# DIG-Beihang/RobustART

Measured on AMD Instinct MI355X. Metric: corrupted+attacked images/sec/node (ResNet-50, PGD-7 + IN-C x5), higher is better.
Workload: dtype bf16x3; 1 GPU; per step and GPU: gaussian_noise sev 1..5 on 256 u8 224x224 images -> normalise -> ResNet-50 eval (1280 img) + PGD-Linf-7 eps 2/255 ResNet-50 eval (256 img); global_batch=256, parallelism=dp1, streams=2

## Files before the change

### include/robustart_hip.h

```cpp
#ifndef ROBUSTART_HIP_H
#define ROBUSTART_HIP_H

#include <stddef.h>
#include <stdint.h>

#ifdef __cplusplus
extern "C" {
#endif

typedef void* rart_stream_t;

typedef enum rart_status {
  RART_OK = 0,
  RART_ERR_INVALID = 1,
  RART_ERR_UNSUPPORTED = 2,
  RART_ERR_WORKSPACE = 3,
  RART_ERR_HIP = 4
} rart_status;

enum {
  RART_GAUSSIAN_NOISE = 0, RART_SHOT_NOISE = 1, RART_IMPULSE_NOISE = 2, RART_DEFOCUS_BLUR = 3,
  RART_GLASS_BLUR = 4, RART_MOTION_BLUR = 5, RART_ZOOM_BLUR = 6, RART_SNOW = 7, RART_FROST = 8,
  RART_FOG = 9, RART_BRIGHTNESS = 10, RART_CONTRAST = 11, RART_ELASTIC_TRANSFORM = 12,
  RART_PIXELATE = 13, RART_JPEG_COMPRESSION = 14, RART_SPECKLE_NOISE = 15, RART_GAUSSIAN_BLUR = 16,
// ... 117 lines not shown
                      float* delta_u, int rows, size_t n, rart_stream_t stream);
int rart_row_count_diff(const float* a, const float* b, float* out, int rows, size_t n, rart_stream_t stream);

int rart_select_rows(float* dst, const float* src, const uint8_t* mask, int batch, size_t n_per_sample,
                     rart_stream_t stream);

int rart_logit_loss(const float* logits, const int64_t* y, const int64_t* y_target, int batch, int classes,
                    int kind, float scale, float* loss_out, float* dlogits_out, int32_t* pred_out,
                    rart_stream_t stream);

typedef struct rart_conv_desc {
  const void* src;
  const void* wgt;
  const float* bias;
  const void* res;
  const void* mask;
  void* dst;
  int32_t batch, grid_h, grid_w;
  int32_t src_h, src_w, src_pix_stride;
  int32_t k_per_tap, n_taps;
  int32_t sy, sx;
  int32_t tap_dy[32], tap_dx[32];
  int64_t tap_src_off[32];
  int32_t n_cols;
  int32_t dst_h, dst_w, dst_sy, dst_sx, dst_oy, dst_ox, dst_pix_stride;
  int32_t flags;
  int32_t n_batched, z_inner, wgt_row_stride, reserved_;
  int64_t src_z_outer, src_z_inner, wgt_z_outer, wgt_z_inner, dst_z_outer, dst_z_inner;
  void* sign_out;
  int64_t dst_pair_off, res_pair_off;
  float* bn_stats_out;
} rart_conv_desc;

int rart_conv_igemm_bf16(const rart_conv_desc* desc_host, rart_stream_t stream);
int rart_igemm_set_bk64_min_k(long long k);
int rart_gemm_small_m_bf16(const void* a, int lda, const void* w, int ldw, const float* bias, void* out, int ldo, int out_is_f32, int m,
                           int n, int k, rart_stream_t stream);
int rart_igemm_set_gemm256(int enable);
int rart_gemm256_supported(long long rows, int k, int n_cols, int src_ld, int dst_ld);

typedef struct rart_gemm_pair_desc {
  const void *a_hi, *a_lo, *w_hi, *w_lo;
  const float* bias;
  const void *res_hi, *res_lo;
  void *dst_hi, *dst_lo;
  void *aux_hi, *aux_lo;
  int M, N, K, lda, ldw, ldc, w_rows;
  int rows_per_image, src_rows_per_image, src_row_off, dst_rows_per_image, dst_row_off;
  int flags, n_batched, z_inner;
  int64_t a_z_outer, a_z_inner, w_z_outer, w_z_inner, c_z_outer, c_z_inner;
  int conv, batch, grid_h, grid_w, src_h, src_w, sy, sx, k_per_tap, n_taps;
  int tap_dy[16], tap_dx[16];
  int dst_h, dst_w, dst_sy, dst_sx, dst_oy, dst_ox;
  const void* mask_bits;
  void* sign_out;
  int tile_n;
  int tile_m;
} rart_gemm_pair_desc;
int rart_gemm_pair_bf16(const rart_gemm_pair_desc* desc_host, rart_stream_t stream);
int rart_gemm_pair_set_schedule(int mode);
int rart_gemm_pair_get_schedule(void);

typedef struct rart_conv_tail_desc {
  const void* a_hi;  const void* a_lo;
  const void* w_hi;  const void* w_lo;
  const void* t_hi;  const void* t_lo;
  const float* bias_mid;
  const float* bias_out;
  const void* mask_mid;  const void* mask_out;
  void* sign_mid;  void* sign_out;
  const void* res_hi;  const void* res_lo;
  void* dst_hi;  void* dst_lo;
  int batch, h, w, c_mid, ldw, relu_mid, relu_out;
  int tap_dy[9], tap_dx[9];
  const void* n_hi;  const void* n_lo;
  const float* bias_next;
  const void* mask_next;
  void* sign_next;
  void* dstn_hi;  void* dstn_lo;
  int relu_next;
} rart_conv_tail_desc;
int rart_conv3x3_tail_pair_supported(int c_mid);
int rart_conv3x3_tail_pair(const rart_conv_tail_desc* desc_host, rart_stream_t stream);

int rart_vit_add_pos_cls_pair(void* x_hi, void* x_lo, const float* cls_pos0, const float* pos, int n, int tokens, int dim,
                              rart_stream_t stream);
int rart_layernorm_pair(const void* x_hi, const void* x_lo, const float* gamma, const float* beta, void* out_hi, void* out_lo, int rows,
                        int dim, int64_t in_row_stride, int64_t out_row_stride, float eps, rart_stream_t stream);
int rart_layernorm_bwd_pair(const void* dy_hi, const void* dy_lo, const void* x_hi, const void* x_lo, const float* gamma,
                            const void* res_hi, const void* res_lo, void* dx_hi, void* dx_lo, int rows, int dim, int64_t dy_row_stride,
                            int64_t x_row_stride, int64_t res_row_stride, int64_t dx_row_stride, float eps, rart_stream_t stream);
int rart_softmax_rows_pair(const float* scores, void* probs_hi, void* probs_lo, int64_t rows, int n_valid, int ld_in, int ld_out,
                           float scale, rart_stream_t stream);
int rart_softmax_bwd_rows_pair(const void* probs_hi, const void* probs_lo, const float* dprobs, void* ds_hi, void* ds_lo, int64_t rows,
                               int n_valid, int ld_p, int ld_dp, int ld_out, float scale, rart_stream_t stream);
int rart_vit_unpatchify_from_f32(const float* dpatches, float* grad, int n, int h, int w, int patch, int64_t ld, const float* std_host,
                                 rart_stream_t stream);
int rart_vit_attention_pair(const void* qkv_hi, const void* qkv_lo, void* out_hi, void* out_lo, int n, int tokens, int heads, int head_dim,
                            rart_stream_t stream);
int rart_vit_attention_bwd_pair(const void* qkv_hi, const void* qkv_lo, const void* out_hi, const void* out_lo, const void* dout_hi,
                                const void* dout_lo, void* dqkv_hi, void* dqkv_lo, float* stats, int n, int tokens, int heads, int head_dim,
                                rart_stream_t stream);

int rart_conv3x3_halo_supported(int channels, int h, int w);
int rart_conv3x3_pack_frag_bf16(const void* w_rows, void* w_frag, int channels, rart_stream_t stream);
int rart_pack_frag_bf16(const void* w_rows, void* w_frag, int rows, int k, rart_stream_t stream);
int rart_conv3x3_halo_bf16(const void* src, const void* wgt, const float* bias, const void* mask_bits, void* sign_out,
                           void* dst, int n, int h, int w, int channels, const int* tap_dy, const int* tap_dx, int relu,
                           rart_stream_t stream);

int rart_bottleneck_fused_supported(int c_io, int c_mid, int h, int w);
int rart_bottleneck_fused_bf16(const void* x, const void* w1, const void* w2, const void* w3, const float* b1, const float* b2,
                               const float* b3, void* m1, void* m2, void* m3, void* out, int n, int h, int w, int c_io,
                               int c_mid, const int* tap_dy, const int* tap_dx, int backward, rart_stream_t stream);

int rart_bottleneck_first_supported(int c_in, int c_mid, int c_out, int h, int w);
int rart_bottleneck_first_bf16(const void* x, const void* w1, const void* w2, const void* w3, const void* w4, const float* b1,
                               const float* b2, const float* b3, void* m1, void* m2, void* m3, void* out, int n, int h, int w,
                               int c_in, int c_mid, int c_out, const int* tap_dy, const int* tap_dx, int backward,
                               rart_stream_t stream);

int rart_bottleneck_s2_fwd_supported(int c_in, int c_mid, int c_out, int h, int w);
int rart_bottleneck_s2_fwd_bf16(const void* x, const void* w1, const void* w2, const void* w3, const void* wd, const float* b1,
                                const float* b2, const float* b3, void* m1, void* m2, void* m3, void* out, int n, int h, int w,
                                int c_in, int c_mid, int c_out, rart_stream_t stream);

int rart_bottleneck_s2_bwd_bf16(const void* g, const void* w3t, const void* w2t, const void* w1t, const void* wdt, const void* m2,
                                const void* m1, const void* m0, void* dx, int n, int h, int w, int c_in, int c_mid, int c_out,
                                rart_stream_t stream);

int rart_bottleneck14_fused_supported(int c_io, int c_mid, int h, int w);
int rart_bottleneck14_fused_bf16(const void* x, const void* w1, const void* w2, const void* w3, const float* b1, const float* b2,
                                 const float* b3, void* m1, void* m2, void* m3, void* out, int n, int h, int w, int c_io,
                                 int c_mid, const int* tap_dy, const int* tap_dx, int backward, rart_stream_t stream);

int rart_bottleneck28_fused_supported(int c_io, int c_mid, int h, int w);
int rart_bottleneck28_fused_bf16(const void* x, const void* w1, const void* w2, const void* w3, const float* b1, const float* b2,
                                 const float* b3, void* m1, void* m2, void* m3, void* out, int n, int h, int w, int c_io,
                                 int c_mid, const int* tap_dy, const int* tap_dx, int backward, rart_stream_t stream);

int rart_bottleneck7_fused_supported(int c_io, int c_mid, int h, int w);
int rart_bottleneck7_fused_bf16(const void* x, const void* w1, const void* w2, const void* w3, const float* b1, const float* b2,
                                const float* b3, void* m1, void* m2, void* m3, void* out, int n, int h, int w, int c_io,
                                int c_mid, const int* tap_dy, const int* tap_dx, int backward, rart_stream_t stream);

int rart_engine_prep_input(const void* src, int src_is_u8, void* hi, void* lo, int n, int h, int w,
                           const float* mean_host, const float* std_host, rart_stream_t stream);
int rart_engine_maxpool(const void* in, void* out, void* argmax_out, int n, int h, int w, int c,
                        rart_stream_t stream);
int rart_engine_maxpool_keep(const void* in, void* out, void* argmax_out, void* sign_out, int n, int h, int w, int c,
                             rart_stream_t stream);
int rart_engine_maxpool_bwd(const void* y, const void* argmax, const void* dpool, void* dz, int n, int h, int w,
                            int c, rart_stream_t stream);
int rart_engine_avgpool(const void* in, void* out, int n, int hw, int c, rart_stream_t stream);
int rart_engine_avgpool_bwd(const void* y, const void* dpool, void* dz, int n, int hw, int c, rart_stream_t stream);
int rart_engine_stem_col2im(const void* patches, float* grad, int n, int h, int w, int patch_cols,
                            const float* std_host, rart_stream_t stream);
int rart_engine_maxpool_pair(const void* in_hi, long long in_lo_off, void* out_hi, long long out_lo_off, void* argmax_out,
                             void* sign_out, int n, int h, int w, int c, rart_stream_t stream);
int rart_engine_maxpool_bwd_pair(const void* argmax, const void* dpool_hi, long long dpool_lo_off, void* dz_hi,
                                 long long dz_lo_off, int n, int h, int w, int c, rart_stream_t stream);
int rart_engine_avgpool_pair(const void* in_hi, long long in_lo_off, void* out_hi, long long out_lo_off, int n, int hw, int c,
                             rart_stream_t stream);
int rart_engine_avgpool_bwd_pair(const void* y_sign_bits, const void* dpool_hi, long long dpool_lo_off, void* dz_hi,
                                 long long dz_lo_off, int n, int hw, int c, rart_stream_t stream);
int rart_f32_to_pair_rows(const float* src, void* dst_hi, long long dst_lo_off, int rows, int cols, int dst_cols,
// ... 132 lines not shown
```

### robustart_amd/_lib.py

```python
import ctypes
import os

_HERE = os.path.dirname(os.path.abspath(__file__))
LIB_PATH = os.path.join(_HERE, 'lib', 'librobustart_hip.so')

c_void_p, c_int, c_size_t, c_u64, c_float = (ctypes.c_void_p, ctypes.c_int, ctypes.c_size_t,
                                              ctypes.c_uint64, ctypes.c_float)
c_double = ctypes.c_double

ABI_VERSION = 110

SIGNATURES = {
    'rart_version': (c_int, []),
    'rart_last_error_string': (ctypes.c_char_p, []),
    'rart_corruption_name': (ctypes.c_char_p, [c_int]),
    'rart_corrupt_workspace_bytes': (c_size_t, [c_int, c_int, c_int, c_int, c_int]),
    'rart_corrupt_u8': (c_int, [c_void_p, c_void_p, c_int, c_int, c_int, c_int, c_int, c_u64, c_u64,
                                ctypes.POINTER(c_void_p), c_int, c_void_p, c_size_t, c_void_p]),
    'rart_stencil_fixed_point_info': (c_int, [c_int, c_int, c_void_p, c_void_p, c_size_t]),
    'rart_noise_multi_u8': (c_int, [c_void_p, ctypes.POINTER(c_void_p), c_int, c_int, c_int, c_int, c_int, ctypes.POINTER(c_int),
                                    ctypes.POINTER(c_u64), c_u64, c_void_p]),
    'rart_frost_textures_u8': (c_int, [c_void_p, c_void_p, c_int, c_int, c_int, c_int, c_void_p, c_int, c_int, c_int, ctypes.POINTER(c_int),
                                       c_u64, c_u64, c_void_p]),
    'rart_pil_resize_workspace_bytes': (c_size_t, [c_int] * 10),
# ... 23 lines not shown
                               c_void_p, c_void_p, c_size_t, c_void_p]),
    'rart_apgd_step': (c_int, [c_void_p, c_void_p, c_void_p, c_void_p, c_void_p, c_int, c_size_t, c_int,
                               c_float, c_float, c_void_p, c_size_t, c_void_p]),
    'rart_square_init_linf': (c_int, [c_void_p, c_void_p, c_int, c_int, c_int, c_int, c_float, c_u64, c_u64, c_void_p, c_void_p,
                                      c_void_p]),
    'rart_rng_signs_f32': (c_int, [c_void_p, c_int, c_int, c_u64, c_u64, c_void_p, c_int, ctypes.c_uint32, c_void_p]),
    'rart_rng_normal_rows_f32': (c_int, [c_void_p, c_int, c_size_t, c_u64, c_void_p, c_int, c_void_p]),
    'rart_square_propose_linf': (c_int, [c_void_p, c_void_p, c_void_p, c_int, c_int, c_int, c_int, c_float, c_int, c_int,
                                         c_int, c_void_p, c_void_p]),
    'rart_fab_project_linf': (c_int, [c_void_p, c_void_p, c_void_p, c_void_p, c_void_p, c_int, c_size_t, c_void_p]),
    'rart_row_dot': (c_int, [c_void_p, c_void_p, c_void_p, c_int, c_size_t, c_void_p]),
    'rart_row_absmax_diff': (c_int, [c_void_p, c_void_p, c_void_p, c_int, c_size_t, c_void_p]),
    'rart_eot_accumulate': (c_int, [c_void_p, c_void_p, c_size_t, c_int, c_float, c_void_p]),
    'rart_square_init_lp': (c_int, [c_void_p, c_void_p, c_int, c_int, c_int, c_int, c_float, c_int, c_int, c_int, c_int, c_int, c_void_p,
                                    c_void_p, c_void_p, c_void_p]),
    'rart_square_propose_lp': (c_int, [c_void_p, c_void_p, c_void_p, c_int, c_int, c_int, c_int, c_float, c_int, c_int, c_int, c_int, c_int,
                                       c_int, c_void_p, c_void_p, c_void_p]),
    'rart_fab_project': (c_int, [c_void_p, c_void_p, c_void_p, c_void_p, c_void_p, c_int, c_size_t, c_int, c_void_p]),
    'rart_row_norm_diff': (c_int, [c_void_p, c_void_p, c_void_p, c_int, c_size_t, c_int, c_void_p]),
    'rart_fab_update': (c_int, [c_void_p, c_void_p, c_void_p, c_void_p, c_void_p, c_int, c_size_t, c_float, c_void_p]),
    'rart_fab_backoff': (c_int, [c_void_p, c_void_p, c_void_p, c_int, c_size_t, c_float, c_void_p]),
    'rart_l1_project': (c_int, [c_void_p, c_void_p, c_void_p, c_int, c_size_t, c_float, c_int, c_int, c_void_p]),
    'rart_row_kth_abs': (c_int, [c_void_p, c_void_p, c_void_p, c_int, c_size_t, c_void_p]),
    'rart_apgd_l1_move': (c_int, [c_void_p, c_void_p, c_void_p, c_void_p, c_void_p, c_void_p, c_int, c_size_t, c_void_p]),
    'rart_row_count_diff': (c_int, [c_void_p, c_void_p, c_void_p, c_int, c_size_t, c_void_p]),
    'rart_select_rows': (c_int, [c_void_p, c_void_p, c_void_p, c_int, c_size_t, c_void_p]),
    'rart_logit_loss': (c_int, [c_void_p, c_void_p, c_void_p, c_int, c_int, c_int, c_float, c_void_p,
                                c_void_p, c_void_p, c_void_p]),
    'rart_conv_igemm_bf16': (c_int, [c_void_p, c_void_p]),
    'rart_conv3x3_halo_supported': (c_int, [c_int, c_int, c_int]),
    'rart_conv3x3_pack_frag_bf16': (c_int, [c_void_p, c_void_p, c_int, c_void_p]),
    'rart_pack_frag_bf16': (c_int, [c_void_p, c_void_p, c_int, c_int, c_void_p]),
    'rart_conv3x3_halo_bf16': (c_int, [c_void_p, c_void_p, c_void_p, c_void_p, c_void_p, c_void_p, c_int, c_int, c_int, c_int,
                                       ctypes.POINTER(c_int), ctypes.POINTER(c_int), c_int, c_void_p]),
    'rart_bottleneck28_fused_supported': (c_int, [c_int, c_int, c_int, c_int]),
    'rart_bottleneck28_fused_bf16': (c_int, [c_void_p] * 11 + [c_int] * 5 + [ctypes.POINTER(c_int), ctypes.POINTER(c_int), c_int,
                                             c_void_p]),
    'rart_bottleneck7_fused_supported': (c_int, [c_int, c_int, c_int, c_int]),
    'rart_bottleneck7_fused_bf16': (c_int, [c_void_p] * 11 + [c_int] * 5 + [ctypes.POINTER(c_int), ctypes.POINTER(c_int), c_int,
                                            c_void_p]),
    'rart_bottleneck_s2_fwd_supported': (c_int, [c_int] * 5),
    'rart_bottleneck_s2_fwd_bf16': (c_int, [c_void_p] * 12 + [c_int] * 6 + [c_void_p]),
    'rart_bottleneck_s2_bwd_bf16': (c_int, [c_void_p] * 9 + [c_int] * 6 + [c_void_p]),
    'rart_bottleneck14_fused_supported': (c_int, [c_int, c_int, c_int, c_int]),
    'rart_bottleneck14_fused_bf16': (c_int, [c_void_p] * 11 + [c_int] * 5 + [ctypes.POINTER(c_int), ctypes.POINTER(c_int), c_int,
                                             c_void_p]),
    'rart_bottleneck_fused_supported': (c_int, [c_int, c_int, c_int, c_int]),
    'rart_bottleneck_first_supported': (c_int, [c_int] * 5),
    'rart_bottleneck_first_bf16': (c_int, [c_void_p] * 12 + [c_int] * 6 + [ctypes.POINTER(c_int), ctypes.POINTER(c_int), c_int,
                                           c_void_p]),
    'rart_bottleneck_fused_bf16': (c_int, [c_void_p] * 11 + [c_int] * 5 + [ctypes.POINTER(c_int), ctypes.POINTER(c_int), c_int,
                                           c_void_p]),
    'rart_igemm_set_bk64_min_k': (c_int, [ctypes.c_longlong]),
    'rart_gemm_small_m_bf16': (c_int, [c_void_p, c_int, c_void_p, c_int, c_void_p, c_void_p, c_int, c_int, c_int, c_int, c_int, c_void_p]),
    'rart_igemm_set_gemm256': (c_int, [c_int]),
    'rart_gemm256_supported': (c_int, [ctypes.c_longlong, c_int, c_int, c_int, c_int]),
    'rart_gemm_pair_bf16': (c_int, [c_void_p, c_void_p]),
    'rart_copy_calibration': (c_int, [c_void_p, c_void_p, ctypes.c_size_t, c_int, c_void_p]),
    'rart_gemm_pair_set_schedule': (c_int, [c_int]),
    'rart_gemm_pair_get_schedule': (c_int, []),
    'rart_pack_jobs_bf16': (c_int, [c_void_p, c_int, c_int, c_void_p]),
    'rart_vit_add_pos_cls_pair': (c_int, [c_void_p, c_void_p, c_void_p, c_void_p, c_int, c_int, c_int, c_void_p]),
    'rart_layernorm_pair': (c_int, [c_void_p] * 6 + [c_int, c_int, ctypes.c_int64, ctypes.c_int64, c_float, c_void_p]),
    'rart_layernorm_bwd_pair': (c_int, [c_void_p] * 9 + [c_int, c_int] + [ctypes.c_int64] * 4 + [c_float, c_void_p]),
    'rart_softmax_rows_pair': (c_int, [c_void_p, c_void_p, c_void_p, ctypes.c_int64, c_int, c_int, c_int, c_float, c_void_p]),
    'rart_softmax_bwd_rows_pair': (c_int, [c_void_p] * 5 + [ctypes.c_int64, c_int, c_int, c_int, c_int, c_float, c_void_p]),
    'rart_vit_attention_pair': (c_int, [c_void_p, c_void_p, c_void_p, c_void_p, c_int, c_int, c_int, c_int, c_void_p]),
    'rart_vit_attention_bwd_pair': (c_int, [c_void_p] * 9 + [c_int, c_int, c_int, c_int, c_void_p]),
    'rart_vit_unpatchify_from_f32': (c_int, [c_void_p, c_void_p, c_int, c_int, c_int, c_int, ctypes.c_int64, ctypes.POINTER(c_float), c_void_p]),
    'rart_engine_prep_input': (c_int, [c_void_p, c_int, c_void_p, c_void_p, c_int, c_int, c_int, c_void_p, c_void_p,
                                       c_void_p]),
    'rart_engine_maxpool': (c_int, [c_void_p, c_void_p, c_void_p, c_int, c_int, c_int, c_int, c_void_p]),
    'rart_engine_maxpool_keep': (c_int, [c_void_p, c_void_p, c_void_p, c_void_p, c_int, c_int, c_int, c_int, c_void_p]),
    'rart_engine_maxpool_bwd': (c_int, [c_void_p, c_void_p, c_void_p, c_void_p, c_int, c_int, c_int, c_int, c_void_p]),
    'rart_engine_avgpool': (c_int, [c_void_p, c_void_p, c_int, c_int, c_int, c_void_p]),
    'rart_engine_avgpool_bwd': (c_int, [c_void_p, c_void_p, c_void_p, c_int, c_int, c_int, c_void_p]),
    'rart_engine_stem_col2im': (c_int, [c_void_p, c_void_p, c_int, c_int, c_int, c_int, c_void_p, c_void_p]),
    'rart_engine_stem_fwd_fused': (c_int, [c_void_p, c_int, c_void_p, c_int, c_void_p, c_void_p, c_void_p, c_void_p, c_int, c_int,
                                           c_int, c_void_p, c_void_p, c_void_p]),
    'rart_wgrad_direct_supported': (c_int, [c_int, c_int, c_int]),
    'rart_wgrad_direct_bf16': (c_int, [c_void_p, c_void_p, c_void_p] + [c_int] * 10 + [c_void_p, c_void_p, c_int, c_int, c_int, c_void_p]),
    'rart_conv3x3_tail_pair_supported': (c_int, [c_int]),
    'rart_conv3x3_tail_pair': (c_int, [c_void_p, c_void_p]),
    'rart_engine_stem_fwd_fused_pair': (c_int, [c_void_p, c_int] + [c_void_p] * 7 + [c_int, c_int, c_int, c_void_p, c_void_p, c_void_p]),
    'rart_engine_stem_bwd_fused_pair': (c_int, [c_void_p] * 6 + [c_int, c_int, c_int, c_void_p, c_void_p]),
    'rart_engine_stem_bwd_fused': (c_int, [c_void_p, c_void_p, c_void_p, c_void_p, c_int, c_int, c_int, c_void_p, c_void_p]),
    'rart_engine_maxpool_pair': (c_int, [c_void_p, ctypes.c_longlong, c_void_p, ctypes.c_longlong, c_void_p, c_void_p, c_int, c_int, c_int, c_int, c_void_p]),
    'rart_engine_maxpool_bwd_pair': (c_int, [c_void_p, c_void_p, ctypes.c_longlong, c_void_p, ctypes.c_longlong, c_int, c_int, c_int, c_int, c_void_p]),
    'rart_engine_avgpool_pair': (c_int, [c_void_p, ctypes.c_longlong, c_void_p, ctypes.c_longlong, c_int, c_int, c_int, c_void_p]),
    'rart_engine_avgpool_bwd_pair': (c_int, [c_void_p, c_void_p, ctypes.c_longlong, c_void_p, ctypes.c_longlong, c_int, c_int, c_int, c_void_p]),
    'rart_f32_to_pair_rows': (c_int, [c_void_p, c_void_p, ctypes.c_longlong, c_int, c_int, c_int, c_void_p]),
    'rart_engine_stem_col2im_f32': (c_int, [c_void_p, c_void_p, c_int, c_int, c_int, c_int, c_void_p, c_void_p]),
    'rart_f32_to_bf16_rows': (c_int, [c_void_p, c_void_p, c_int, c_int, c_int, c_void_p]),
    'rart_cnx_dwconv_ln_bf16': (c_int, [c_void_p] * 7 + [c_int] * 4 + [c_float, c_void_p]),
    'rart_cnx_dwconv_ln_pair': (c_int, [c_void_p] * 10 + [c_int] * 4 + [c_float, c_void_p]),
    'rart_cnx_dwconv_bwd_bf16': (c_int, [c_void_p] * 4 + [c_int] * 4 + [c_void_p]),
    'rart_cnx_dwconv_bwd_pair': (c_int, [c_void_p] * 7 + [c_int] * 4 + [c_void_p]),
    'rart_cnx_pool_bwd_bf16': (c_int, [c_void_p, c_void_p, c_int, c_int, c_int, c_void_p]),
    'rart_cnx_pool_bwd_pair': (c_int, [c_void_p] * 4 + [c_int, c_int, c_int, c_void_p]),
    'rart_cnx_patchify': (c_int, [c_void_p, c_int, c_void_p, c_void_p, c_int, c_int, c_int, c_int, c_int, c_void_p, c_void_p, c_void_p]),
    'rart_cnx_dwconv_wgrad_workspace_bytes': (c_size_t, [c_int] * 4),
    'rart_cnx_dwconv_wgrad_bf16': (c_int, [c_void_p] * 4 + [c_int] * 6 + [c_void_p, c_size_t, c_void_p]),
    'rart_cnx_layer_scale_fwd_bf16': (c_int, [c_void_p] * 4 + [ctypes.c_longlong, c_int, c_void_p]),
    'rart_cnx_layer_scale_bwd_workspace_bytes': (c_size_t, [ctypes.c_longlong, c_int]),
    'rart_cnx_layer_scale_bwd_bf16': (c_int, [c_void_p] * 6 + [ctypes.c_longlong, c_int, c_int, c_void_p, c_size_t, c_void_p]),
    'rart_cnx_grn_stats_bf16': (c_int, [c_void_p] * 2 + [c_int] * 3 + [c_void_p]),
    'rart_cnx_grn_stats_pair': (c_int, [c_void_p] * 3 + [c_int] * 3 + [c_void_p]),
    'rart_cnx_grn_apply_bf16': (c_int, [c_void_p] * 5 + [c_int] * 3 + [c_float, c_void_p]),
    'rart_cnx_grn_apply_pair': (c_int, [c_void_p] * 7 + [c_int] * 3 + [c_float, c_void_p]),
    'rart_cnx_grn_bwd_reduce_bf16': (c_int, [c_void_p] * 4 + [c_int] * 3 + [c_void_p]),
    'rart_cnx_grn_bwd_reduce_pair': (c_int, [c_void_p] * 6 + [c_int] * 3 + [c_void_p]),
    'rart_cnx_grn_bwd_apply_bf16': (c_int, [c_void_p] * 7 + [c_int] * 3 + [c_float, c_void_p]),
    'rart_cnx_grn_bwd_apply_pair': (c_int, [c_void_p] * 11 + [c_int] * 3 + [c_float, c_void_p]),
    'rart_cnx_grn_param_grad_workspace_bytes': (c_size_t, [c_int] * 2),
    'rart_cnx_grn_bwd_reduce_train_bf16': (c_int, [c_void_p] * 7 + [c_int] * 3 + [c_float, c_int, c_void_p, c_size_t, c_void_p]),
    'rart_vit_patchify': (c_int, [c_void_p, c_int, c_void_p, c_void_p, c_int, c_int, c_int, c_int, c_void_p, c_void_p,
                                  c_void_p]),
    'rart_vit_add_pos_cls': (c_int, [c_void_p, c_void_p, c_void_p, c_int, c_int, c_int, c_void_p]),
    'rart_layernorm_bf16': (c_int, [c_void_p, c_void_p, c_void_p, c_void_p, c_int, c_int, ctypes.c_int64, ctypes.c_int64,
                                    c_float, c_void_p]),
    'rart_softmax_rows_bf16': (c_int, [c_void_p, c_void_p, ctypes.c_int64, c_int, c_int, c_int, c_float, c_void_p]),
    'rart_vit_attention': (c_int, [c_void_p, c_void_p, c_int, c_int, c_int, c_int, c_void_p]),
    'rart_vit_attention_bwd': (c_int, [c_void_p, c_void_p, c_void_p, c_void_p, c_int, c_int, c_int, c_int, c_void_p]),
    'rart_vit_transpose_v': (c_int, [c_void_p, c_void_p, c_int, c_int, c_int, c_int, c_int, c_int, c_int, c_void_p]),
    'rart_gelu_bf16': (c_int, [c_void_p, c_void_p, c_size_t, c_void_p]),
    'rart_gelu_bwd_bf16': (c_int, [c_void_p, c_void_p, c_void_p, c_size_t, c_void_p]),
    'rart_layernorm_bwd_bf16': (c_int, [c_void_p, c_void_p, c_void_p, c_void_p, c_void_p, c_int, c_int, ctypes.c_int64,
                                        ctypes.c_int64, ctypes.c_int64, ctypes.c_int64, c_float, c_void_p]),
    'rart_softmax_bwd_rows_bf16': (c_int, [c_void_p, c_void_p, c_void_p, ctypes.c_int64, c_int, c_int, c_int, c_int, c_float,
                                           c_void_p]),
    'rart_vit_unpatchify_f32': (c_int, [c_void_p, c_void_p, c_int, c_int, c_int, c_int, ctypes.c_int64,
                                        ctypes.POINTER(c_float), c_void_p]),
    'rart_layernorm_bwd_workspace_bytes': (c_size_t, [c_int]),
    'rart_layernorm_bwd_full_bf16': (c_int, [c_void_p, c_void_p, c_void_p, c_void_p, c_void_p, c_int, c_int, ctypes.c_int64,
                                             ctypes.c_int64, ctypes.c_int64, ctypes.c_int64, c_float, c_void_p, c_void_p, c_int,
                                             c_void_p, c_size_t, c_void_p]),
    'rart_colsum_workspace_bytes': (c_size_t, [c_int, c_int]),
    'rart_colsum_bf16': (c_int, [c_void_p, ctypes.c_int64, c_int, c_int, c_void_p, c_int, c_void_p, c_size_t, c_void_p]),
    'rart_sgd_step_f32': (c_int, [c_void_p, c_void_p, c_void_p, c_void_p, c_size_t, c_double, c_double, c_double, c_int,
                                  c_double, c_double, c_int, c_void_p]),
    'rart_adamw_step_f32': (c_int, [c_void_p, c_void_p, c_void_p, c_void_p, c_void_p, c_size_t, c_double, c_double,
                                    c_double, c_double, c_double, c_int, c_double, c_double, c_int, c_void_p]),
    'rart_ema_update_f32': (c_int, [c_void_p, c_void_p, c_size_t, c_double, c_void_p]),
    'rart_label_smooth_ce_f32': (c_int, [c_void_p, c_void_p, c_int, c_int, c_double, c_double, c_void_p, c_void_p,
                                         c_void_p]),
    'rart_bn_workspace_bytes': (c_size_t, [c_size_t, c_int]),
    'rart_bn_train_forward_bf16': (c_int, [c_void_p, c_void_p, c_void_p, c_void_p, c_size_t, c_int, c_void_p, c_void_p, c_void_p,
                                           c_void_p, c_double, c_double, c_int, c_void_p, c_void_p, c_void_p, c_void_p, c_int, c_void_p,
                                           c_size_t, c_void_p]),
    'rart_bn_train_backward_bf16': (c_int, [c_void_p, c_void_p, c_int, c_void_p, c_void_p, c_void_p, c_size_t, c_int, c_void_p,
                                            c_void_p, c_void_p, c_void_p, c_void_p, c_int, c_void_p, c_void_p, c_size_t,
                                            c_void_p]),
    'rart_transpose_gather_bf16': (c_int, [c_void_p, c_void_p, c_int, c_int, c_int, c_int, c_int, c_int, c_int, c_int,
                                           c_int, ctypes.POINTER(c_int), ctypes.POINTER(c_int), ctypes.c_longlong,
                                           c_int, c_int, c_void_p]),
    'rart_wgrad_reduce_f32': (c_int, [c_void_p, c_int, c_int, c_int, c_int, c_int, c_int, c_void_p, c_int, c_void_p]),
    'rart_pack_conv_weight_bf16': (c_int, [c_void_p, c_void_p, c_void_p, c_int, c_int, c_int, c_int, c_int,
                                           ctypes.POINTER(c_int), ctypes.POINTER(c_int), c_int, c_int, c_void_p]),
}


class ConvDesc(ctypes.Structure):
    _fields_ = [('src', c_void_p), ('wgt', c_void_p), ('bias', c_void_p), ('res', c_void_p), ('mask', c_void_p),
                ('dst', c_void_p),
                ('batch', ctypes.c_int32), ('grid_h', ctypes.c_int32), ('grid_w', ctypes.c_int32),
                ('src_h', ctypes.c_int32), ('src_w', ctypes.c_int32), ('src_pix_stride', ctypes.c_int32),
# ... 113 lines not shown
```

### robustart_amd/csrc/conv_tail_pair.hip

```cpp
#include "rart_common.h"
#include "rart_lds_dma.h"

typedef __attribute__((ext_vector_type(8))) __bf16 bf16x8;
typedef __attribute__((ext_vector_type(16))) float f32x16;

namespace {
constexpr int CT_TM = 128;
constexpr int CT_LDE = 68;
constexpr int CT_PLANE_A = CT_TM * 64;
constexpr int CT_NLD = 144;
constexpr int CT_WREG = 2 * 32 * CT_NLD;
static_assert(CT_WREG >= 32 * CT_LDE * 4, "the staging must fit the wave's region");

struct ConvTailDev {
  const uint16_t *a_hi, *a_lo, *w_hi, *w_lo, *t_hi, *t_lo;
  const float *bias_mid, *bias_out;
  const uint8_t *mask_mid, *mask_out;
  uint8_t *sign_mid, *sign_out;
  const uint16_t *res_hi, *res_lo;
  uint16_t *dst_hi, *dst_lo;
  int M, H, W, ldw, relu_mid, relu_out;
  int tap_dy[9], tap_dx[9];
  uint32_t w_magic, w_shift, h_magic, h_shift;
  const uint16_t *n_hi, *n_lo;
  const float* bias_next;
  const uint8_t* mask_next;
  uint8_t* sign_next;
  uint16_t *dstn_hi, *dstn_lo;
  int relu_next;
};
typedef __attribute__((ext_vector_type(4))) uint32_t ct_u4;
__device__ __forceinline__ uint4 ct_nt_load(const uint16_t* p) {
  const ct_u4 v = __builtin_nontemporal_load(reinterpret_cast<const ct_u4*>(p));
  return make_uint4(v[0], v[1], v[2], v[3]);
}
__device__ __forceinline__ void ct_nt_store(uint16_t* p, const uint4& v) {
  ct_u4 w = {v.x, v.y, v.z, v.w};
  __builtin_nontemporal_store(w, reinterpret_cast<ct_u4*>(p));
}
__device__ __forceinline__ uint32_t ct_fastdiv(uint32_t n, uint32_t magic, uint32_t shift) { return (uint32_t)(((uint64_t)n * magic) >> shift); }

__device__ __forceinline__ uint32_t ct_pack_bf16x2(float lo, float hi) {
  typedef __attribute__((ext_vector_type(2))) float f2_t;
  typedef __attribute__((ext_vector_type(2))) __bf16 b2_t;
  f2_t f = {lo, hi};
  return __builtin_bit_cast(uint32_t, __builtin_convertvector(f, b2_t));
}
__device__ __forceinline__ void ct_split8(const float* v, uint4& hi, uint4& lo) {
  uint32_t h[4], l[4];
#pragma unroll
  for (int j = 0; j < 4; ++j) {
    h[j] = ct_pack_bf16x2(v[2 * j], v[2 * j + 1]);
    l[j] = ct_pack_bf16x2(v[2 * j] - __uint_as_float(h[j] << 16), v[2 * j + 1] - __uint_as_float(h[j] & 0xFFFF0000u));
  }
  hi = make_uint4(h[0], h[1], h[2], h[3]);
  lo = make_uint4(l[0], l[1], l[2], l[3]);
}
__device__ __forceinline__ void ct_join8(const uint4& hi, const uint4& lo, float* v) {
  const uint32_t h[4] = {hi.x, hi.y, hi.z, hi.w}, l[4] = {lo.x, lo.y, lo.z, lo.w};
#pragma unroll
  for (int j = 0; j < 4; ++j) {
    v[2 * j] = __uint_as_float(h[j] << 16) + __uint_as_float(l[j] << 16);
    v[2 * j + 1] = __uint_as_float(h[j] & 0xFFFF0000u) + __uint_as_float(l[j] & 0xFFFF0000u);
  }
}
__device__ __forceinline__ uint32_t ct_sign_byte(const uint4& v) {
  const uint32_t hw[4] = {v.x, v.y, v.z, v.w};
  uint32_t sb = 0;
#pragma unroll
  for (int j = 0; j < 4; ++j) {
    sb |= ((short)(hw[j] & 0xFFFFu) > 0 ? 1u : 0u) << (2 * j);
    sb |= ((short)(hw[j] >> 16) > 0 ? 1u : 0u) << (2 * j + 1);
  }
  return sb;
}

template <int NJ>
__device__ __forceinline__ void ct_pointwise_frags(const f32x16* acc, const uint32_t* mw, bool relu, int h, uint4* fh, uint4* fl) {
#pragma unroll
  for (int j = 0; j < NJ; ++j)
#pragma unroll
    for (int ge = 0; ge < 4; ge += 2) {
      uint32_t eh[2], el[2], oh[2], ol[2];
#pragma unroll
// ... 234 lines not shown
        if (d.res_hi) {
          float rv[8];
          ct_join8(rh[q], rl[q], rv);
#pragma unroll
          for (int j = 0; j < 8; ++j) v[j] += rv[j];
        }
#pragma unroll
        for (int j = 0; j < 8; ++j)
          if (!((mb[q] >> j) & 1u)) v[j] = 0.f;
        if (relu_out) {
#pragma unroll
          for (int j = 0; j < 8; ++j) v[j] = fmaxf(v[j], 0.f);
        }
        uint4 ph, pl;
        ct_split8(v, ph, pl);
        ct_nt_store(d.dst_hi + e, ph);
        ct_nt_store(d.dst_lo + e, pl);
        if (d.sign_out) d.sign_out[e >> 3] = (uint8_t)ct_sign_byte(ph);
        oph[q] = ph;
        opl[q] = pl;
      }
    }
    __builtin_amdgcn_fence(__ATOMIC_RELEASE, "wavefront");
    __builtin_amdgcn_wave_barrier();
    if (NEXT) {
#pragma unroll
      for (int q = 0; q < 4; ++q) {
        *reinterpret_cast<uint4*>(wreg + (q * 8 + rw) * CT_NLD + cw * 16) = oph[q];
        *reinterpret_cast<uint4*>(wreg + 32 * CT_NLD + (q * 8 + rw) * CT_NLD + cw * 16) = opl[q];
      }
      __builtin_amdgcn_fence(__ATOMIC_RELEASE, "wavefront");
      __builtin_amdgcn_wave_barrier();
      __builtin_amdgcn_fence(__ATOMIC_ACQUIRE, "wavefront");
      bf16x8 xh[4], xl[4];
#pragma unroll
      for (int s = 0; s < 4; ++s) {
        xh[s] = *reinterpret_cast<const bf16x8*>(wreg + fr * CT_NLD + s * 32 + h * 16);
        xl[s] = *reinterpret_cast<const bf16x8*>(wreg + 32 * CT_NLD + fr * CT_NLD + s * 32 + h * 16);
      }
      const uint4* nh_base = reinterpret_cast<const uint4*>(d.n_hi) + lane;
      const uint4* nl_base = reinterpret_cast<const uint4*>(d.n_lo) + lane;
#pragma unroll
      for (int j = 0; j < NJ; ++j) {
        uint4 nh[4], nl[4];
#pragma unroll
        for (int s = 0; s < 4; ++s) {
          nh[s] = nh_base[((c * NJ + j) * 4 + s) * 64];
          nl[s] = nl_base[((c * NJ + j) * 4 + s) * 64];
        }
#pragma unroll
        for (int s = 0; s < 4; ++s) {
          const bf16x8 wh = __builtin_bit_cast(bf16x8, nh[s]), wl = __builtin_bit_cast(bf16x8, nl[s]);
          accn[j] = __builtin_amdgcn_mfma_f32_32x32x16_bf16(wh, xl[s], accn[j], 0, 0, 0);
          accn[j] = __builtin_amdgcn_mfma_f32_32x32x16_bf16(wl, xh[s], accn[j], 0, 0, 0);
          accn[j] = __builtin_amdgcn_mfma_f32_32x32x16_bf16(wh, xh[s], accn[j], 0, 0, 0);
        }
      }
      __builtin_amdgcn_fence(__ATOMIC_RELEASE, "wavefront");
      __builtin_amdgcn_wave_barrier();
    }
  }
  if (NEXT) {
    uint32_t mw[NJ];
#pragma unroll
    for (int j = 0; j < NJ; ++j) mw[j] = 0xFFFFFFFFu;
    if (d.mask_next && p_ok) {
      const uint32_t* mp = reinterpret_cast<const uint32_t*>(d.mask_next + (size_t)p * (C / 8));
#pragma unroll
      for (int j = 0; j < NJ; ++j) mw[j] = mp[j];
    }
    uint4 fh[KS], fl[KS];
    ct_pointwise_frags<NJ>(accn, mw, d.relu_next != 0, h, fh, fl);
    if (p_ok) {
#pragma unroll
      for (int s = 0; s < KS; ++s) {
        ct_nt_store(d.dstn_hi + (size_t)p * C + 16 * s + 8 * h, fh[s]);
        ct_nt_store(d.dstn_lo + (size_t)p * C + 16 * s + 8 * h, fl[s]);
        if (d.sign_next) d.sign_next[(size_t)p * (C / 8) + 2 * s + h] = (uint8_t)ct_sign_byte(fh[s]);
      }
    }
  }
}

void ct_magic(uint32_t dv, uint32_t& mg, uint32_t& sh) {
  uint32_t l = 0;
  while ((1ull << l) < dv) ++l;
  sh = 31 + l;
  mg = (uint32_t)(((1ull << sh) + dv - 1) / dv);
}
}

extern "C" int rart_conv3x3_tail_pair_supported(int c_mid) { return (c_mid == 64 || c_mid == 128) ? 1 : 0; }

extern "C" int rart_conv3x3_tail_pair(const rart_conv_tail_desc* t, rart_stream_t stream) {
  RART_CHECK_ARG(t != nullptr, "rart_conv3x3_tail_pair: null descriptor");
  RART_CHECK_ARG(t->a_hi && t->a_lo && t->w_hi && t->w_lo && t->t_hi && t->t_lo && t->dst_hi && t->dst_lo,
                 "rart_conv3x3_tail_pair: null operand plane");
  RART_CHECK_ARG(t->c_mid == 64 || t->c_mid == 128, "rart_conv3x3_tail_pair: c_mid must be 64 or 128 (layer1 / layer2)");
  RART_CHECK_ARG(t->batch > 0 && t->h > 0 && t->w > 0, "rart_conv3x3_tail_pair: empty geometry");
  RART_CHECK_ARG((t->res_hi == nullptr) == (t->res_lo == nullptr), "rart_conv3x3_tail_pair: the skip is a pair: both planes or none");
  RART_CHECK_ARG(t->ldw % 8 == 0 && t->ldw >= 9 * t->c_mid, "rart_conv3x3_tail_pair: ldw must cover 9 taps x c_mid and keep 16-byte alignment");
  const long long M = (long long)t->batch * t->h * t->w;
  RART_CHECK_ARG(M * 4 * t->c_mid < (1ll << 31), "rart_conv3x3_tail_pair: tensors must stay below 2^31 elements (split the batch)");
  ConvTailDev d;
  d.a_hi = (const uint16_t*)t->a_hi; d.a_lo = (const uint16_t*)t->a_lo; d.w_hi = (const uint16_t*)t->w_hi; d.w_lo = (const uint16_t*)t->w_lo;
  d.t_hi = (const uint16_t*)t->t_hi; d.t_lo = (const uint16_t*)t->t_lo;
  d.bias_mid = t->bias_mid; d.bias_out = t->bias_out;
  d.mask_mid = (const uint8_t*)t->mask_mid; d.mask_out = (const uint8_t*)t->mask_out;
  d.sign_mid = (uint8_t*)t->sign_mid; d.sign_out = (uint8_t*)t->sign_out;
  d.res_hi = (const uint16_t*)t->res_hi; d.res_lo = (const uint16_t*)t->res_lo;
  d.dst_hi = (uint16_t*)t->dst_hi; d.dst_lo = (uint16_t*)t->dst_lo;
  d.M = (int)M; d.H = t->h; d.W = t->w; d.ldw = t->ldw; d.relu_mid = t->relu_mid; d.relu_out = t->relu_out;
  for (int i = 0; i < 9; ++i) { d.tap_dy[i] = t->tap_dy[i]; d.tap_dx[i] = t->tap_dx[i]; }
  const bool next = t->n_hi != nullptr;
  RART_CHECK_ARG(!next || (t->n_lo && t->dstn_hi && t->dstn_lo), "rart_conv3x3_tail_pair: the neighbour's reduction needs both table planes and its destination pair");
  d.n_hi = (const uint16_t*)t->n_hi; d.n_lo = (const uint16_t*)t->n_lo; d.bias_next = t->bias_next; d.mask_next = (const uint8_t*)t->mask_next;
  d.sign_next = (uint8_t*)t->sign_next; d.dstn_hi = (uint16_t*)t->dstn_hi; d.dstn_lo = (uint16_t*)t->dstn_lo; d.relu_next = t->relu_next;
  ct_magic((uint32_t)d.W, d.w_magic, d.w_shift);
  ct_magic((uint32_t)d.H, d.h_magic, d.h_shift);
  const dim3 grid((uint32_t)((M + CT_TM - 1) / CT_TM));
  hipStream_t st = (hipStream_t)stream;
  if (t->c_mid == 64) {
    if (next) hipLaunchKernelGGL((k_conv3x3_tail_pair<64, true>), grid, dim3(256), 0, st, d);
    else hipLaunchKernelGGL((k_conv3x3_tail_pair<64, false>), grid, dim3(256), 0, st, d);
  } else {
    if (next) hipLaunchKernelGGL((k_conv3x3_tail_pair<128, true>), grid, dim3(256), 0, st, d);
    else hipLaunchKernelGGL((k_conv3x3_tail_pair<128, false>), grid, dim3(256), 0, st, d);
  }
  RART_CHECK_LAUNCH("rart_conv3x3_tail_pair");
  return RART_OK;
}
```

Baseline: 8341 images/s.

## Add wide 256-position tile variant for layer1 fused conv3x3 tail kernel

Adds a new kernel for the c_mid=64 fused 3x3-conv + 1x1 tail path in which each wave handles two 32-row position blocks (256 or 224 positions per workgroup) instead of the 128-position tile. Each weight fragment loaded from LDS is reused across two position blocks, which cuts weight traffic and launch count per position. It also adds XCD-aware tile remapping. An env/API-selectable variant defaults to using wide tiles only for launches without the fused neighbour reduction. The cost is more registers, which limits occupancy to two blocks, plus a larger LDS footprint.

```diff
diff --git a/include/robustart_hip.h b/include/robustart_hip.h
--- a/include/robustart_hip.h
+++ b/include/robustart_hip.h
@@ -223,6 +223,8 @@
 } rart_conv_tail_desc;
 int rart_conv3x3_tail_pair_supported(int c_mid);
 int rart_conv3x3_tail_pair(const rart_conv_tail_desc* desc_host, rart_stream_t stream);
+int rart_conv3x3_tail_pair_set_variant(int variant);
+int rart_conv3x3_tail_pair_get_variant(void);
 
 int rart_vit_add_pos_cls_pair(void* x_hi, void* x_lo, const float* cls_pos0, const float* pos, int n, int tokens, int dim,
                               rart_stream_t stream);
diff --git a/robustart_amd/_lib.py b/robustart_amd/_lib.py
--- a/robustart_amd/_lib.py
+++ b/robustart_amd/_lib.py
@@ -129,6 +129,8 @@
     'rart_wgrad_direct_bf16': (c_int, [c_void_p, c_void_p, c_void_p] + [c_int] * 10 + [c_void_p, c_void_p, c_int, c_int, c_int, c_void_p]),
     'rart_conv3x3_tail_pair_supported': (c_int, [c_int]),
     'rart_conv3x3_tail_pair': (c_int, [c_void_p, c_void_p]),
+    'rart_conv3x3_tail_pair_set_variant': (c_int, [c_int]),
+    'rart_conv3x3_tail_pair_get_variant': (c_int, []),
     'rart_engine_stem_fwd_fused_pair': (c_int, [c_void_p, c_int] + [c_void_p] * 7 + [c_int, c_int, c_int, c_void_p, c_void_p, c_void_p]),
     'rart_engine_stem_bwd_fused_pair': (c_int, [c_void_p] * 6 + [c_int, c_int, c_int, c_void_p, c_void_p]),
     'rart_engine_stem_bwd_fused': (c_int, [c_void_p, c_void_p, c_void_p, c_void_p, c_int, c_int, c_int, c_void_p, c_void_p]),
diff --git a/robustart_amd/csrc/conv_tail_pair.hip b/robustart_amd/csrc/conv_tail_pair.hip
--- a/robustart_amd/csrc/conv_tail_pair.hip
+++ b/robustart_amd/csrc/conv_tail_pair.hip
@@ -1,5 +1,6 @@
 #include "rart_common.h"
 #include "rart_lds_dma.h"
+#include <stdlib.h>
 
 typedef __attribute__((ext_vector_type(8))) __bf16 bf16x8;
 typedef __attribute__((ext_vector_type(16))) float f32x16;
@@ -400,13 +401,383 @@
   }
 }
 
+constexpr int CW_TM = 256;
+constexpr int CW_PLANE_A = CW_TM * 64;
+
+constexpr int CW_STAGE = 2 * CW_PLANE_A + 2 * 64 * 64;
+static_assert(8 * CT_WREG <= 2 * CW_STAGE, "the waves' two epilogue regions must fit the tile buffers");
+
+template <bool NEXT, int TM, int NB>
+__device__ __forceinline__ void ct_wide_body(const ConvTailDev& d, uint8_t* lds, int wave) {
+  constexpr int C = 64, NJ = 2, KS = 4, NOUT = 4 * C, NC = NOUT / 64;
+  constexpr int KT = 18;
+  constexpr int PLANE_B = C * 64, STAGE = CW_STAGE;
+  constexpr int PIECES = TM / 16;
+  constexpr int nb = NB;
+  const int lane = threadIdx.x & 63;
+  uint32_t tile;
+  {
+    const uint32_t nbk = gridDim.x, bid = blockIdx.x, xcd = bid & 7u, slot = bid >> 3, q = nbk >> 3, r = nbk & 7u;
+    tile = (xcd < r ? xcd * (q + 1u) : r * (q + 1u) + (xcd - r) * q) + slot;
+  }
+  const int m0 = (int)tile * TM;
+
+  uint32_t avoff[4], nok[4] = {0u, 0u, 0u, 0u};
+  int tap_min = 0;
+  for (int t = 0; t < 9; ++t) tap_min = min(tap_min, (d.tap_dy[t] * d.W + d.tap_dx[t]) * (C * 2));
+  const int tapreg = lane < 9 ? (d.tap_dy[lane] * d.W + d.tap_dx[lane]) * (C * 2) - tap_min : 0;
+#pragma unroll
+  for (int q = 0; q < 4; ++q) {
+    const int r = 16 * (wave + 4 * q) + (lane >> 2);
+    const int cs = ((lane & 3) ^ ((r >> 2) & 3)) * 16;
+    const int m = m0 + r;
+    const bool ok = r < TM && m < d.M;
+    const uint32_t mm = ok ? (uint32_t)m : 0u;
+    const uint32_t t = ct_fastdiv(mm, d.w_magic, d.w_shift);
+    const int ax = (int)(mm - t * (uint32_t)d.W);
+    const int n = (int)ct_fastdiv(t, d.h_magic, d.h_shift);
+    const int ay = (int)(t - (uint32_t)n * (uint32_t)d.H);
+    avoff[q] = (uint32_t)((n * d.H * d.W + ay * d.W + ax) * (C * 2) + cs);
+    for (int t2 = 0; t2 < 9; ++t2) {
+      const int iy = ay + d.tap_dy[t2], ix = ax + d.tap_dx[t2];
+      if (!(ok && (unsigned)iy < (unsigned)d.H && (unsigned)ix < (unsigned)d.W)) nok[q] |= 1u << t2;
+    }
+  }
+  uint32_t wvoff;
+  {
+    const int r = 16 * wave + (lane >> 2);
+    wvoff = (uint32_t)((r * d.ldw + (((lane & 3) ^ ((r >> 2) & 3)) * 8)) * 2);
+  }
+  const rart_srd_t srd_ah = rart_dma_srd(reinterpret_cast<const char*>(d.a_hi) + tap_min), srd_al = rart_dma_srd(reinterpret_cast<const char*>(d.a_lo) + tap_min);
+  const rart_srd_t srd_wh = rart_dma_srd(d.w_hi), srd_wl = rart_dma_srd(d.w_lo);
+  const uint32_t lds_base = (uint32_t)(uintptr_t)(__attribute__((address_space(3))) uint8_t*)lds;
+#define RART_CW_ISSUE(KT_, BUF)                                                                                 \
+  {                                                                                                             \
+    const uint32_t st_ = lds_base + (BUF)*STAGE;                                                                \
+    const int kt_ = (KT_);                                                                                      \
+    const int tap_ = kt_ >> 1;                                                                                  \
+    const uint32_t so_ = (uint32_t)(__builtin_amdgcn_readlane(tapreg, tap_) + (kt_ - (tap_ << 1)) * 64);        \
+    _Pragma("unroll") for (int q = 0; q < 4; ++q) {                                                             \
+      if (wave + 4 * q < PIECES) {                                                                              \
+        const uint32_t vo_ = avoff[q] | ((uint32_t)__builtin_amdgcn_sbfe(nok[q], tap_, 1) & RART_DMA_OOR);      \
+        rart_dma_load16(vo_, srd_ah, so_, st_ + (wave + 4 * q) * 1024);                                         \
+        rart_dma_load16(vo_, srd_al, so_, st_ + CW_PLANE_A + (wave + 4 * q) * 1024);                            \
+      }                                                                                                         \
+    }                                                                                                           \
+    rart_dma_load16(wvoff, srd_wh, (uint32_t)kt_ * 64u, st_ + 2 * CW_PLANE_A + wave * 1024);                    \
+    rart_dma_load16(wvoff, srd_wl, (uint32_t)kt_ * 64u, st_ + 2 * CW_PLANE_A + PLANE_B + wave * 1024);          \
+  }
+  const int fr = lane & 31, h = lane >> 5;
+  uint32_t xo[2];
+#pragma unroll
+  for (int ks = 0; ks < 2; ++ks) xo[ks] = (uint32_t)(fr * 64 + (((2 * ks + h) ^ ((fr >> 2) & 3)) << 4));
+  f32x16 acc[2][NJ];
+#pragma unroll
+  for (int j = 0; j < NJ; ++j)
+#pragma unroll
+    for (int g = 0; g < 4; ++g) {
+      float4 bv = make_float4(0.f, 0.f, 0.f, 0.f);
+      if (d.bias_mid) bv = *reinterpret_cast<const float4*>(d.bias_mid + j * 32 + 8 * g + 4 * h);
+#pragma unroll
+      for (int pb = 0; pb < 2; ++pb) {
+        acc[pb][j][4 * g] = bv.x; acc[pb][j][4 * g + 1] = bv.y; acc[pb][j][4 * g + 2] = bv.z; acc[pb][j][4 * g + 3] = bv.w;
+      }
+    }
+  RART_CW_ISSUE(0, 0)
+  rart_dma_wait<0>();
+  __syncthreads();
+  for (int kt = 0; kt < KT; ++kt) {
+    const int buf = kt & 1;
+    if (kt + 1 < KT) RART_CW_ISSUE(kt + 1, buf ^ 1)
+    const uint8_t* Pb = lds + buf * STAGE + (wave * 64) * 64;
+    const uint8_t* Wb = lds + buf * STAGE + 2 * CW_PLANE_A;
+#pragma unroll
+    for (int ks = 0; ks < 2; ++ks) {
+      bf16x8 wh[NJ], wl[NJ];
+#pragma unroll
+      for (int j = 0; j < NJ; ++j) {
+        wh[j] = *reinterpret_cast<const bf16x8*>(Wb + j * 32 * 64 + xo[ks]);
+        wl[j] = *reinterpret_cast<const bf16x8*>(Wb + PLANE_B + j * 32 * 64 + xo[ks]);
+      }
+#pragma unroll
+      for (int pb = 0; pb < 2; ++pb) {
+        if (pb < nb) {
+          const bf16x8 ph = *reinterpret_cast<const bf16x8*>(Pb + pb * 32 * 64 + xo[ks]);
+          const bf16x8 pl = *reinterpret_cast<const bf16x8*>(Pb + CW_PLANE_A + pb * 32 * 64 + xo[ks]);
+#pragma unroll
+          for (int j = 0; j < NJ; ++j) {
+            acc[pb][j] = __builtin_amdgcn_mfma_f32_32x32x16_bf16(wh[j], pl, acc[pb][j], 0, 0, 0);
+            acc[pb][j] = __builtin_amdgcn_mfma_f32_32x32x16_bf16(wl[j], ph, acc[pb][j], 0, 0, 0);
+            acc[pb][j] = __builtin_amdgcn_mfma_f32_32x32x16_bf16(wh[j], ph, acc[pb][j], 0, 0, 0);
+          }
+        }
+      }
+    }
+    rart_dma_wait<0>();
+    __syncthreads();
+  }
+#undef RART_CW_ISSUE
+
+  int pp0[2];
+  bool pok[2];
+  bf16x8 a2h[2][KS], a2l[2][KS];
+#pragma unroll
+  for (int pb = 0; pb < 2; ++pb) {
+    pp0[pb] = m0 + wave * 64 + pb * 32;
+    pok[pb] = pb < nb && pp0[pb] + fr < d.M;
+    if (pb < nb) {
+      const int p = pp0[pb] + fr;
+      uint32_t mw[NJ];
+#pragma unroll
+      for (int j = 0; j < NJ; ++j) mw[j] = 0xFFFFFFFFu;
+      if (d.mask_mid && pok[pb]) {
+        const uint32_t* mp = reinterpret_cast<const uint32_t*>(d.mask_mid + (size_t)p * (C / 8));
+#pragma unroll
+        for (int j = 0; j < NJ; ++j) mw[j] = mp[j];
+      }
+      uint4 fh[KS], fl[KS];
+      ct_pointwise_frags<NJ>(acc[pb], mw, d.relu_mid != 0, h, fh, fl);
+#pragma unroll
+      for (int s = 0; s < KS; ++s) {
+        a2h[pb][s] = __builtin_bit_cast(bf16x8, fh[s]);
+        a2l[pb][s] = __builtin_bit_cast(bf16x8, fl[s]);
+        if (d.sign_mid && pok[pb]) d.sign_mid[(size_t)p * (C / 8) + 2 * s + h] = (uint8_t)ct_sign_byte(fh[s]);
+      }
+    }
+  }
+
+  uint8_t* const wreg = lds + wave * 2 * CT_WREG;
+  const int cw = lane & 7, rw = lane >> 3;
+  f32x16 accn[2][NEXT ? NJ : 1];
+  if (NEXT) {
+#pragma unroll
+    for (int j = 0; j < NJ; ++j)
+#pragma unroll
+      for (int g = 0; g < 4; ++g) {
+        float4 bv = make_float4(0.f, 0.f, 0.f, 0.f);
+        if (d.bias_next) bv = *reinterpret_cast<const float4*>(d.bias_next + j * 32 + 8 * g + 4 * h);
+#pragma unroll
+        for (int pb = 0; pb < 2; ++pb) {
+          accn[pb][j][4 * g] = bv.x; accn[pb][j][4 * g + 1] = bv.y; accn[pb][j][4 * g + 2] = bv.z; accn[pb][j][4 * g + 3] = bv.w;
+        }
+      }
+  }
+  const uint4* th_base = reinterpret_cast<const uint4*>(d.t_hi) + lane;
+  const uint4* tl_base = reinterpret_cast<const uint4*>(d.t_lo) + lane;
+  const bool relu_out = d.relu_out != 0;
+#pragma unroll 1
+  for (int c = 0; c < NC; ++c) {
+    int eo[2][4];
+    uint4 rh[2][4], rl[2][4];
+    uint32_t mb[2][4];
+#define RART_CW_SKIP(PB)                                                         \
+    _Pragma("unroll") for (int q = 0; q < 4; ++q) {                             \
+      const int pp = pp0[PB] + q * 8 + rw;                                       \
+      eo[PB][q] = -1;                                                            \
+      rh[PB][q] = rl[PB][q] = make_uint4(0, 0, 0, 0);                            \
+      mb[PB][q] = 0xFFu;                                                         \
+      if (PB < nb && pp < d.M) {                                                 \
+        const int e = pp * NOUT + c * 64 + cw * 8;                               \
+        eo[PB][q] = e;                                                           \
+        if (d.res_hi) {                                                          \
+          rh[PB][q] = ct_nt_load(d.res_hi + e);                                  \
+          rl[PB][q] = ct_nt_load(d.res_lo + e);                                  \
+        }                                                                        \
+        if (d.mask_out) mb[PB][q] = d.mask_out[e >> 3];                          \
+      }                                                                          \
+    }
+    RART_CW_SKIP(0)
+    if (!NEXT) RART_CW_SKIP(1)
+#pragma unroll
+    for (int b = 0; b < 2; ++b) {
+      f32x16 acc2[2];
+#pragma unroll
+      for (int g = 0; g < 4; ++g) {
+        float4 bv = make_float4(0.f, 0.f, 0.f, 0.f);
+        if (d.bias_out) bv = *reinterpret_cast<const float4*>(d.bias_out + c * 64 + b * 32 + 8 * g + 4 * h);
+#pragma unroll
+        for (int pb = 0; pb < 2; ++pb) {
+          acc2[pb][4 * g] = bv.x; acc2[pb][4 * g + 1] = bv.y; acc2[pb][4 * g + 2] = bv.z; acc2[pb][4 * g + 3] = bv.w;
+        }
+      }
+      uint4 th[KS], tl[KS];
+#pragma unroll
+      for (int s = 0; s < KS; ++s) {
+        th[s] = th_base[((c * 2 + b) * KS + s) * 64];
+        tl[s] = tl_base[((c * 2 + b) * KS + s) * 64];
+      }
+#pragma unroll
+      for (int s = 0; s < KS; ++s) {
+        const bf16x8 wh = __builtin_bit_cast(bf16x8, th[s]), wl = __builtin_bit_cast(bf16x8, tl[s]);
+#pragma unroll
+        for (int pb = 0; pb < 2; ++pb) {
+          if (pb < nb) {
+            acc2[pb] = __builtin_amdgcn_mfma_f32_32x32x16_bf16(wh, a2l[pb][s], acc2[pb], 0, 0, 0);
+            acc2[pb] = __builtin_amdgcn_mfma_f32_32x32x16_bf16(wl, a2h[pb][s], acc2[pb], 0, 0, 0);
+            acc2[pb] = __builtin_amdgcn_mfma_f32_32x32x16_bf16(wh, a2h[pb][s], acc2[pb], 0, 0, 0);
+          }
+        }
+      }
+#pragma unroll
+      for (int pb = 0; pb < 2; ++pb) {
+        if (pb < nb) {
+          float* sE = reinterpret_cast<float*>(wreg + pb * CT_WREG);
+#pragma unroll
+          for (int g = 0; g < 4; ++g)
+            *reinterpret_cast<float4*>(sE + fr * CT_LDE + b * 32 + 8 * g + 4 * h) =
+                make_float4(acc2[pb][4 * g], acc2[pb][4 * g + 1], acc2[pb][4 * g + 2], acc2[pb][4 * g + 3]);
+        }
+      }
+    }
+    __builtin_amdgcn_fence(__ATOMIC_RELEASE, "wavefront");
+    __builtin_amdgcn_wave_barrier();
+    __builtin_amdgcn_fence(__ATOMIC_ACQUIRE, "wavefront");
+#pragma unroll
+    for (int pb = 0; pb < 2; ++pb) {
+      if (NEXT && pb == 1) RART_CW_SKIP(1)
+      if (pb < nb) {
+        uint8_t* const rg = wreg + pb * CT_WREG;
+        const float* sE = reinterpret_cast<const float*>(rg);
+        uint4 oph[4], opl[4];
+#pragma unroll
+        for (int q = 0; q < 4; ++q) {
+          const int r = q * 8 + rw;
+          const float4 v0 = *reinterpret_cast<const float4*>(sE + r * CT_LDE + cw * 8);
+          const float4 v1 = *reinterpret_cast<const float4*>(sE + r * CT_LDE + cw * 8 + 4);
+          const int e = eo[pb][q];
+          oph[q] = opl[q] = make_uint4(0, 0, 0, 0);
+          if (e >= 0) {
+            float v[8] = {v0.x, v0.y, v0.z, v0.w, v1.x, v1.y, v1.z, v1.w};
+            if (d.res_hi) {
+              float rv[8];
+              ct_join8(rh[pb][q], rl[pb][q], rv);
+#pragma unroll
+              for (int j = 0; j < 8; ++j) v[j] += rv[j];
+            }
+#pragma unroll
+            for (int j = 0; j < 8; ++j)
+              if (!((mb[pb][q] >> j) & 1u)) v[j] = 0.f;
+            if (relu_out) {
+#pragma unroll
+              for (int j = 0; j < 8; ++j) v[j] = fmaxf(v[j], 0.f);
+            }
+            uint4 ph, pl;
+            ct_split8(v, ph, pl);
+            ct_nt_store(d.dst_hi + e, ph);
+            ct_nt_store(d.dst_lo + e, pl);
+            if (d.sign_out) d.sign_out[e >> 3] = (uint8_t)ct_sign_byte(ph);
+            oph[q] = ph;
+            opl[q] = pl;
+          }
+        }
+        if (NEXT) {
+          __builtin_amdgcn_fence(__ATOMIC_RELEASE, "wavefront");
+          __builtin_amdgcn_wave_barrier();
+#pragma unroll
+          for (int q = 0; q < 4; ++q) {
+            *reinterpret_cast<uint4*>(rg + (q * 8 + rw) * CT_NLD + cw * 16) = oph[q];
+            *reinterpret_cast<uint4*>(rg + 32 * CT_NLD + (q * 8 + rw) * CT_NLD + cw * 16) = opl[q];
+          }
+        }
+      }
+    }
+#undef RART_CW_SKIP
+    __builtin_amdgcn_fence(__ATOMIC_RELEASE, "wavefront");
+    __builtin_amdgcn_wave_barrier();
+    if (NEXT) {
+      __builtin_amdgcn_fence(__ATOMIC_ACQUIRE, "wavefront");
+      const uint4* nh_base = reinterpret_cast<const uint4*>(d.n_hi) + lane;
+      const uint4* nl_base = reinterpret_cast<const uint4*>(d.n_lo) + lane;
+#pragma unroll
+      for (int j = 0; j < NJ; ++j) {
+        uint4 nh[4], nl[4];
+#pragma unroll
+        for (int s = 0; s < 4; ++s) {
+          nh[s] = nh_base[((c * NJ + j) * 4 + s) * 64];
+          nl[s] = nl_base[((c * NJ + j) * 4 + s) * 64];
+        }
+#pragma unroll
+        for (int pb = 0; pb < 2; ++pb) {
+          if (pb < nb) {
+            const uint8_t* const rg = wreg + pb * CT_WREG;
+#pragma unroll
+            for (int s = 0; s < 4; ++s) {
+              const bf16x8 xh = *reinterpret_cast<const bf16x8*>(rg + fr * CT_NLD + s * 32 + h * 16);
+              const bf16x8 xl = *reinterpret_cast<const bf16x8*>(rg + 32 * CT_NLD + fr * CT_NLD + s * 32 + h * 16);
+              const bf16x8 wh = __builtin_bit_cast(bf16x8, nh[s]), wl = __builtin_bit_cast(bf16x8, nl[s]);
+              accn[pb][j] = __builtin_amdgcn_mfma_f32_32x32x16_bf16(wh, xl, accn[pb][j], 0, 0, 0);
+              accn[pb][j] = __builtin_amdgcn_mfma_f32_32x32x16_bf16(wl, xh, accn[pb][j], 0, 0, 0);
+              accn[pb][j] = __builtin_amdgcn_mfma_f32_32x32x16_bf16(wh, xh, accn[pb][j], 0, 0, 0);
+            }
+          }
+        }
+      }
+      __builtin_amdgcn_fence(__ATOMIC_RELEASE, "wavefront");
+      __builtin_amdgcn_wave_barrier();
+    }
+  }
+  if (NEXT) {
+#pragma unroll
+    for (int pb = 0; pb < 2; ++pb) {
+      if (pb < nb) {
+        const int p = pp0[pb] + fr;
+        uint32_t mw[NJ];
+#pragma unroll
+        for (int j = 0; j < NJ; ++j) mw[j] = 0xFFFFFFFFu;
+        if (d.mask_next && pok[pb]) {
+          const uint32_t* mp = reinterpret_cast<const uint32_t*>(d.mask_next + (size_t)p * (C / 8));
+#pragma unroll
+          for (int j = 0; j < NJ; ++j) mw[j] = mp[j];
+        }
+        uint4 fh[KS], fl[KS];
+        ct_pointwise_frags<NJ>(accn[pb], mw, d.relu_next != 0, h, fh, fl);
+        if (pok[pb]) {
+#pragma unroll
+          for (int s = 0; s < KS; ++s) {
+            ct_nt_store(d.dstn_hi + (size_t)p * C + 16 * s + 8 * h, fh[s]);
+            ct_nt_store(d.dstn_lo + (size_t)p * C + 16 * s + 8 * h, fl[s]);
+            if (d.sign_next) d.sign_next[(size_t)p * (C / 8) + 2 * s + h] = (uint8_t)ct_sign_byte(fh[s]);
+          }
+        }
+      }
+    }
+  }
+}
+
+template <bool NEXT, int TM>
+__global__ __launch_bounds__(256, 2) void k_conv3x3_tail_pair_w64(const ConvTailDev d) {
+  static_assert(TM == 256 || TM == 224, "wide tiles are 256 or 224 positions");
+  __shared__ __attribute__((aligned(16))) uint8_t lds[2 * CW_STAGE];
+  const int wave = __builtin_amdgcn_readfirstlane(threadIdx.x >> 6);
+  if (TM == 256 || wave < 3) ct_wide_body<NEXT, TM, 2>(d, lds, wave);
+  else ct_wide_body<NEXT, TM, 1>(d, lds, wave);
+}
+
 void ct_magic(uint32_t dv, uint32_t& mg, uint32_t& sh) {
   uint32_t l = 0;
   while ((1ull << l) < dv) ++l;
   sh = 31 + l;
   mg = (uint32_t)(((1ull << sh) + dv - 1) / dv);
 }
-}
+
+int g_tail_variant = -1;
+int ct_variant() {
+  if (g_tail_variant < 0) {
+    const char* e = getenv("RART_TAIL_VARIANT");
+    g_tail_variant = e ? atoi(e) : 1;
+    if (g_tail_variant < 0 || g_tail_variant > 3) g_tail_variant = 1;
+  }
+  return g_tail_variant;
+}
+}
+
+extern "C" int rart_conv3x3_tail_pair_set_variant(int variant) {
+  RART_CHECK_ARG(variant >= 0 && variant <= 3,
+                 "rart_conv3x3_tail_pair_set_variant: variant must be 0 (128-position tiles), 1 (wide tiles for plain launches), 2 (wide, 256) or 3 (wide, 224)");
+  g_tail_variant = variant;
+  return RART_OK;
+}
+extern "C" int rart_conv3x3_tail_pair_get_variant(void) { return ct_variant(); }
 
 extern "C" int rart_conv3x3_tail_pair_supported(int c_mid) { return (c_mid == 64 || c_mid == 128) ? 1 : 0; }
 
@@ -436,8 +807,22 @@
   d.sign_next = (uint8_t*)t->sign_next; d.dstn_hi = (uint16_t*)t->dstn_hi; d.dstn_lo = (uint16_t*)t->dstn_lo; d.relu_next = t->relu_next;
   ct_magic((uint32_t)d.W, d.w_magic, d.w_shift);
   ct_magic((uint32_t)d.H, d.h_magic, d.h_shift);
+  hipStream_t st = (hipStream_t)stream;
+  const int variant = ct_variant();
+  if (t->c_mid == 64 && (variant >= 2 || (variant == 1 && !next))) {
+    const int tm = variant == 3 ? 224 : 256;
+    const dim3 grid((uint32_t)((M + tm - 1) / tm));
+    if (tm == 256) {
+      if (next) hipLaunchKernelGGL((k_conv3x3_tail_pair_w64<true, 256>), grid, dim3(256), 0, st, d);
+      else hipLaunchKernelGGL((k_conv3x3_tail_pair_w64<false, 256>), grid, dim3(256), 0, st, d);
+    } else {
+      if (next) hipLaunchKernelGGL((k_conv3x3_tail_pair_w64<true, 224>), grid, dim3(256), 0, st, d);
+      else hipLaunchKernelGGL((k_conv3x3_tail_pair_w64<false, 224>), grid, dim3(256), 0, st, d);
+    }
+    RART_CHECK_LAUNCH("rart_conv3x3_tail_pair (wide tiles)");
+    return RART_OK;
+  }
   const dim3 grid((uint32_t)((M + CT_TM - 1) / CT_TM));
-  hipStream_t st = (hipStream_t)stream;
   if (t->c_mid == 64) {
     if (next) hipLaunchKernelGGL((k_conv3x3_tail_pair<64, true>), grid, dim3(256), 0, st, d);
     else hipLaunchKernelGGL((k_conv3x3_tail_pair<64, false>), grid, dim3(256), 0, st, d);
```

After: 8353 images/s (median of 5 runs). No clear change (+0.1%).
